# SHI-Labs/Prompt-Free-Diffusion

Hardware: NVIDIA H100
Metric: 512x512 images/sec @ 50 DDIM steps (higher is better)
Workload: dtype fp16

## Files before the change

### pfd_b200/autokl.py

```python
from __future__ import annotations

from typing import Optional

import torch
import torch.nn as nn

from . import native as nv
from .modules import Container, Conv2d, GroupNorm, pk_conv3, pk_conv3_small, pk_lin, pk_mat, pk_norm


def Normalize(c):
    return GroupNorm(32, c, eps=1e-6, affine=True)


class ResnetBlock(nn.Module):

    def __init__(self, in_channels, out_channels=None):
        super().__init__()
        out_channels = out_channels or in_channels
        self.in_channels, self.out_channels = in_channels, out_channels
        self.norm1 = Normalize(in_channels)
        self.conv1 = Conv2d(in_channels, out_channels, 3, padding=1)
        self.norm2 = Normalize(out_channels)
        self.dropout = nn.Dropout(0.0)
        self.conv2 = Conv2d(out_channels, out_channels, 3, padding=1)
        if in_channels != out_channels:
            self.nin_shortcut = Conv2d(in_channels, out_channels, 1)


class AttnBlock(nn.Module):

    def __init__(self, c):
        super().__init__()
        self.in_channels = c
        self.norm = Normalize(c)
        self.q, self.k, self.v, self.proj_out = Conv2d(c, c, 1), Conv2d(c, c, 1), Conv2d(c, c, 1), Conv2d(c, c, 1)


class _Resample(nn.Module):
    def __init__(self, c, stride):
        super().__init__()
# ... 128 lines not shown
        h = run_vae_resnet(enc.mid.block_1, h)
        h = run_vae_attn(enc.mid.attn_1, h)
        h = run_vae_resnet(enc.mid.block_2, h)
        g, b = pk_norm(enc.norm_out)
        h = nv.groupnorm(h, g, b, enc.norm_out.eps, silu=True)
        w, b = pk_conv3(enc.conv_out)
        h = nv.conv3x3(h, w, b)
        wq, bq = pk_lin(self.quant_conv)
        mom = nv.conv1x1(h, wq, bq)
        zc = self.quant_conv.weight.shape[0] // 2
        if out_posterior:
            return DiagonalGaussianDistribution(mom, zc)
        noise = torch.randn((B, zc, mom.shape[1], mom.shape[2])).to(mom.device)
        return nv.vae_posterior(mom, zc, noise=noise, scale=post_scale, want=("sample",))["sample"]

    @torch.no_grad()
    def decode(self, z: torch.Tensor, pre_scale: float = 1.0) -> torch.Tensor:
        dec = self.decoder
        B, Cz, H, W = z.shape
        nv.gn_reset()
        zc = nv.nchw_to_nhwc(z if z.dtype == torch.float32 else z.to(torch.float16), cpad=8)
        wq, bq = pk_lin(self.post_quant_conv)
        h = nv.linear(zc.reshape(B * H * W, 8), wq, bq, alpha=pre_scale).reshape(B, H, W, 8)
        w, b = cached_conv_in(dec.conv_in, Cz)
        h = nv.conv3x3_im2col(h, w, b)
        h = run_vae_resnet(dec.mid.block_1, h)
        h = run_vae_attn(dec.mid.attn_1, h)
        h = run_vae_resnet(dec.mid.block_2, h)
        for lvl in reversed(range(dec.num_resolutions)):
            up = dec.up[lvl]
            for rb in up.block:
                h = run_vae_resnet(rb, h)
            if lvl != 0:
                w, b = pk_conv3(up.upsample.conv)
                h = nv.conv3x3(nv.upsample2x(h), w, b)
        g, b = pk_norm(dec.norm_out)
        h = nv.groupnorm(h, g, b, dec.norm_out.eps, silu=True)
        w, b = pk_conv3(dec.conv_out)
        h = nv.conv3x3(h, w, b)
        return nv.nhwc_to_nchw(h, dec.out_ch, mul=0.5, add=0.5, lo=0.0, hi=1.0)

    def forward(self, z):
        return self.decode(z)


class DiagonalGaussianDistribution(object):

    def __init__(self, moments: torch.Tensor, zc: int):
        self._mom, self._zc = moments, zc
        o = nv.vae_posterior(moments, zc, want=("mean", "logvar", "std"))
        self.mean, self.logvar, self.std = o["mean"], o["logvar"], o["std"]
        self.deterministic = False

    def sample(self):
        noise = torch.randn(self.mean.shape).to(self.mean.device)
        return nv.vae_posterior(self._mom, self._zc, noise=noise, want=("sample",))["sample"]

    def mode(self):
        return self.mean


def cached_conv_in(conv: Conv2d, cz: int):
    from .modules import cached, fp16

    def build():
        o = conv.weight.shape[0]
        w = torch.zeros((o, 3, 3, 8), device=conv.weight.device, dtype=torch.float16)
        w[..., :cz] = fp16(conv.weight).permute(0, 2, 3, 1)
# ... 3 lines not shown
```

### pfd_b200/csrc/gemm_tc.cu

```cuda
#include <cuda.h>
#include <cuda_fp16.h>
#include <cuda_runtime.h>
#include <math.h>
#include <string.h>

#include "../../include/pfd_b200.h"
#include "common.h"
#include "ptx.cuh"
#include "wgmma.cuh"

namespace pfd {

constexpr int BM = 128;
constexpr int BK = 64;
constexpr int WG_K = 16;
constexpr int GEMM_THREADS = 384;
constexpr int STAGE_A_BYTES = BM * BK * 2;
constexpr int SMEM_BUDGET = 232448;
constexpr int SMEM_FIXED = 1024 + 256;

struct alignas(64) GemmParams {
  CUtensorMap tmA[PFD_MAX_SEG];
  CUtensorMap tmB;
  int nseg;
  int taps[PFD_MAX_SEG];
  int chunks[PFD_MAX_SEG];
  int a_c[PFD_MAX_SEG];
  int stride;
  int tap_off;
  int bw, bh, bn;
  int tiles_w, tiles_h, tiles_nb, n_tiles;
  int W, H, NB, N;
  int b_batched;
  int num_kb;
  int splits;
  int kb_per_split;
  float* ws;
  float alpha;
  int act;
  const __half* bias;
  const __half* rowadd;
  const __half* residual;
  __half* out;
  long long so_n1, so_n0, so_y, so_x, so_c1, so_c0;
  long long rowadd_ld;
  int ndiv, cdiv;
  int vec_ok;
};

constexpr int STORE_THREADS = 96;

template <int BN>
struct GemmCfg {
  static constexpr int STAGE_B_BYTES = BN * BK * 2;
  static constexpr int STAGE_BYTES = STAGE_A_BYTES + STAGE_B_BYTES;
  static constexpr int C_PITCH = BN * 2 + 16;
  static constexpr int C_BYTES = BM * C_PITCH + 2 * BM * 8;
  static constexpr int RAW_STAGES = (SMEM_BUDGET - SMEM_FIXED - C_BYTES) / STAGE_BYTES;
  static constexpr int STAGES = RAW_STAGES > 8 ? 8 : RAW_STAGES;
  static constexpr int SMEM_BYTES = STAGES * STAGE_BYTES + C_BYTES + SMEM_FIXED;
  static constexpr int CONSUMER_REGS = BN >= 256 ? 224 : 208;
  static constexpr int PRODUCER_REGS = BN >= 256 ? 56 : 88;
  static constexpr int STORE_BATCH = BN >= 256 ? 4 : 8;
  static constexpr bool BIAS_EARLY = BN < 256;
// ... 40 lines not shown
  lo = fmaf(lo, alpha, h2lo(bias));
  hi = fmaf(hi, alpha, h2hi(bias));
  if (rowadd) {
    lo += h2lo(ra);
    hi += h2hi(ra);
  }
  if (act != PFD_ACT_NONE) {
    lo = act_apply(lo, act);
    hi = act_apply(hi, act);
  }
}

__device__ __forceinline__ __half2 geglu_pair(const float* v, const float* g, float alpha, uint32_t bv, uint32_t bg) {
  const __half2 a = __floats2half2_rn(fmaf(v[0], alpha, h2lo(bv)), fmaf(v[1], alpha, h2hi(bv)));
  const float2 gf = __half22float2(__floats2half2_rn(fmaf(g[0], alpha, h2lo(bg)), fmaf(g[1], alpha, h2hi(bg))));
  return __hmul2(a, __floats2half2_rn(gelu_sig(gf.x), gelu_sig(gf.y)));
}

struct WorkItem {
  int tile, kb0, kb1, slot;
};
__device__ __forceinline__ bool gemm_work(const GemmParams& p, int wi, int total_tiles, WorkItem& w) {
  const int G = gridDim.x, c = blockIdx.x;
  const int work = c + wi * G;
  if (work >= total_tiles * p.splits) return false;
  w.tile = work % total_tiles;
  w.slot = work / total_tiles;
  w.kb0 = w.slot * p.kb_per_split;
  w.kb1 = min(p.num_kb, w.kb0 + p.kb_per_split);
  return true;
}

struct TileOrigin {
  int x0, y0, n0, lbw, lbh;
};
__device__ __forceinline__ TileOrigin tile_origin(const GemmParams& p, int m_tile) {
  TileOrigin o;
  o.x0 = (m_tile % p.tiles_w) * p.bw;
  o.y0 = ((m_tile / p.tiles_w) % p.tiles_h) * p.bh;
  o.n0 = (m_tile / (p.tiles_w * p.tiles_h)) * p.bn;
  o.lbw = __ffs(p.bw) - 1;
  o.lbh = __ffs(p.bh) - 1;
  return o;
}
struct TileRow {
  int x, y, n;
  bool valid;
};
__device__ __forceinline__ TileRow tile_row(const GemmParams& p, const TileOrigin& o, int row) {
  TileRow r;
  r.x = o.x0 + (row & (p.bw - 1));
  r.y = o.y0 + ((row >> o.lbw) & (p.bh - 1));
  r.n = o.n0 + (row >> (o.lbw + o.lbh));
  r.valid = (r.x < p.W) && (r.y < p.H) && (r.n < p.NB);
  return r;
}
__device__ __forceinline__ long long out_row_off(const GemmParams& p, const TileRow& r) {
  return (long long)(r.n / p.ndiv) * p.so_n1 + (long long)(r.n % p.ndiv) * p.so_n0 + (long long)r.y * p.so_y +
         (long long)r.x * p.so_x;
}
__device__ __forceinline__ long long out_col_off(const GemmParams& p, int c) {
  return p.cdiv >= p.N ? (long long)c * p.so_c0 : (long long)(c / p.cdiv) * p.so_c1 + (long long)(c % p.cdiv) * p.so_c0;
}

template <int BN>
__device__ __forceinline__ void gemm_load_bias(const GemmParams& p, int tile, uint32_t (&bias)[BN / 8]) {
  const int col0 = (tile % p.n_tiles) * BN + 2 * (threadIdx.x & 3);
#pragma unroll
  for (int j = 0; j < BN / 8; ++j) bias[j] = (p.bias && col0 + 8 * j < p.N) ? ldg_h2(p.bias + col0 + 8 * j) : 0u;
}

template <int BN, bool GEGLU>
__device__ __forceinline__ void gemm_stage_tile(const GemmParams& p, const float (&acc)[BN / 2],
                                                const uint32_t (&bias)[BN / 8], int cw, int tile, uint8_t* cbuf) {
  constexpr int C_PITCH = GemmCfg<BN>::C_PITCH;
  const int wl = (threadIdx.x >> 5) & 3, lane = threadIdx.x & 31;
  const int n_tile = tile % p.n_tiles;
  const TileOrigin org = tile_origin(p, tile / p.n_tiles);
  const int n_out = GEGLU ? p.N / 2 : p.N;
  const int col_base = n_tile * (GEGLU ? BN / 2 : BN);
  const int cq = 2 * (lane & 3);
  int rows[2];
  bool valid[2];
  const __half* rowadd_row[2];
#pragma unroll
  for (int i = 0; i < 2; ++i) {
    rows[i] = cw * 64 + wl * 16 + (lane >> 2) + 8 * i;
    const TileRow r = tile_row(p, org, rows[i]);
    valid[i] = r.valid;
    rowadd_row[i] = (p.rowadd && r.valid) ? p.rowadd + (long long)r.n * p.rowadd_ld : nullptr;
  }
  auto put = [&](int i, int c, __half2 h) {
// ... 21 lines not shown
    uint32_t ra[2][JB];
#pragma unroll
    for (int jj = 0; jj < JB; ++jj) {
      const int col = col_base + 8 * (j0 + jj) + cq;
#pragma unroll
      for (int i = 0; i < 2; ++i) ra[i][jj] = (rowadd_row[i] && col < n_out) ? ldg_h2(rowadd_row[i] + col) : 0u;
    }
#pragma unroll
    for (int jj = 0; jj < JB; ++jj) {
      const int j = j0 + jj;
      if (col_base + 8 * j + cq >= n_out) continue;
#pragma unroll
      for (int i = 0; i < 2; ++i) {
        if (!valid[i]) continue;
        float v0 = acc[4 * j + 2 * i], v1 = acc[4 * j + 2 * i + 1];
        epi_pair(v0, v1, alpha, bias[j], rowadd_row[i] != nullptr, ra[i][jj], act);
        put(i, 8 * j + cq, __floats2half2_rn(v0, v1));
      }
    }
  }
}

template <int BN, bool GEGLU>
__device__ __forceinline__ void gemm_store_tile(const GemmParams& p, int tile, const uint8_t* cbuf, long long* rowoff,
                                                uint32_t c_full, uint32_t parity) {
  constexpr int C_PITCH = GemmCfg<BN>::C_PITCH;
  constexpr int STORE_BATCH = GemmCfg<BN>::STORE_BATCH;
  constexpr int CPR = (GEGLU ? BN / 2 : BN) / 8;
  constexpr int RPP = STORE_THREADS / CPR;
  constexpr int NPASS = (BM + RPP - 1) / RPP;
  const int t = threadIdx.x - 32;
  const int n_tile = tile % p.n_tiles;
  const TileOrigin org = tile_origin(p, tile / p.n_tiles);
  const bool line_tile = p.bw == BM;
  if (!line_tile) {
#pragma unroll 1
    for (int row = t; row < BM; row += STORE_THREADS) {
      const TileRow r = tile_row(p, org, row);
      rowoff[row] = r.valid ? out_row_off(p, r) : -1;
    }
    asm volatile("bar.sync 2, %0;" ::"n"(STORE_THREADS) : "memory");
  }
  const int ch = t % CPR, r0 = t / CPR;
  const int col = n_tile * CPR * 8 + 8 * ch;
  const bool col_ok = r0 < RPP && col < (GEGLU ? p.N / 2 : p.N);
  const long long col_off = out_col_off(p, col);
  const bool add_res = p.residual && !GEGLU;
  const uint8_t* const src = cbuf + r0 * C_PITCH + ch * 16;

  auto store_rows = [&](auto row_off) {
    uint4 res[STORE_BATCH];
    auto load_batch = [&](int pass0) {
#pragma unroll
      for (int b = 0; b < STORE_BATCH; ++b) {
        const int row = r0 + (pass0 + b) * RPP;
        const long long off = (col_ok && row < BM) ? row_off(row) : -1;
        if (off >= 0) res[b] = __ldg(reinterpret_cast<const uint4*>(p.residual + off));
      }
    };
    if (add_res) load_batch(0);
    mbar_wait(c_full, parity);
#pragma unroll 1
    for (int pass0 = 0; pass0 < NPASS; pass0 += STORE_BATCH) {
#pragma unroll
      for (int b = 0; b < STORE_BATCH; ++b) {
        const int row = r0 + (pass0 + b) * RPP;
        const long long off = (col_ok && row < BM) ? row_off(row) : -1;
        if (off < 0) continue;
        uint4 v = *reinterpret_cast<const uint4*>(src + (pass0 + b) * (RPP * C_PITCH));
        if (add_res) {
          __half2* h = reinterpret_cast<__half2*>(&v);
          const __half2* r = reinterpret_cast<const __half2*>(&res[b]);
#pragma unroll
          for (int k = 0; k < 4; ++k) h[k] = __hadd2(h[k], r[k]);
        }
        *reinterpret_cast<uint4*>(p.out + off) = v;
      }
      if (add_res && pass0 + STORE_BATCH < NPASS) load_batch(pass0 + STORE_BATCH);
    }
  };

  if (line_tile) {
    const int rows_in = p.W - org.x0;
    TileRow first;
    first.x = org.x0; first.y = org.y0; first.n = org.n0;
    const long long base = out_row_off(p, first) + col_off;
    const long long so_x = p.so_x;
    store_rows([&](int row) { return row < rows_in ? base + row * so_x : -1ll; });
  } else {
    store_rows([&](int row) {
      const long long ro = rowoff[row];
      return ro >= 0 ? ro + col_off : -1ll;
    });
  }
}

template <int BN>
__device__ __forceinline__ void gemm_epilogue(const GemmParams& p, const float (&acc)[BN / 2], int cw, int tile,
                                              int split, int m_tiles) {
  const int wl = (threadIdx.x >> 5) & 3, lane = threadIdx.x & 31;
  const int n_tile = tile % p.n_tiles;
  const int m_tile = tile / p.n_tiles;
  const TileOrigin org = tile_origin(p, m_tile);
  const bool geglu = (p.act == PFD_ACT_GEGLU);
  const int n_out = geglu ? p.N / 2 : p.N;
  const int col_base = n_tile * (geglu ? BN / 2 : BN);
  const int cq = 2 * (lane & 3);
  int rows[2];
  bool valid[2];
  long long row_off[2];
  const __half* rowadd_row[2];
#pragma unroll
  for (int i = 0; i < 2; ++i) {
    const int row = cw * 64 + wl * 16 + (lane >> 2) + 8 * i;
    rows[i] = row;
    const TileRow r = tile_row(p, org, row);
    valid[i] = r.valid;
    row_off[i] = out_row_off(p, r);
    rowadd_row[i] = (p.rowadd && valid[i]) ? p.rowadd + (long long)r.n * p.rowadd_ld : nullptr;
// ... 68 lines not shown
  constexpr int STAGES = Cfg::STAGES;
  extern __shared__ uint8_t smem_raw[];

  const uint32_t raw_addr = smem_u32(smem_raw);
  const uint32_t base = (raw_addr + 1023u) & ~1023u;
  const uint32_t smemA = base;
  const uint32_t smemB = base + STAGES * STAGE_A_BYTES;
  const uint32_t cbuf_off = base - raw_addr + STAGES * Cfg::STAGE_BYTES;
  uint8_t* const cbuf = smem_raw + cbuf_off;
  long long* const rowoff = reinterpret_cast<long long*>(cbuf + BM * Cfg::C_PITCH);
  const uint32_t bars = base + STAGES * Cfg::STAGE_BYTES + Cfg::C_BYTES;
  auto full_bar = [&](int s) { return bars + 8u * s; };
  auto empty_bar = [&](int s) { return bars + 8u * (STAGES + s); };
  const uint32_t c_full = bars + 16u * STAGES, c_empty = c_full + 8u;

  const int wg = threadIdx.x >> 7;
  const bool staged = p.vec_ok && p.splits == 1;

  if (threadIdx.x == 0) {
    for (int s = 0; s < p.nseg; ++s) tma_prefetch_desc(&p.tmA[s]);
    tma_prefetch_desc(&p.tmB);
    for (int s = 0; s < STAGES; ++s) {
      mbar_init(full_bar(s), 1);
      mbar_init(empty_bar(s), 8);
    }
    mbar_init(c_full, 8);
    mbar_init(c_empty, STORE_THREADS / 32);
    mbar_fence_init();
  }
  __syncthreads();
  pdl_wait();
  pdl_launch_dependents();

  const int m_tiles = p.tiles_w * p.tiles_h * p.tiles_nb;
  const int total_tiles = m_tiles * p.n_tiles;

  if (wg == 0) {
    setmaxnreg_dec<Cfg::PRODUCER_REGS>();
    if (threadIdx.x >= 32 && staged) {
      uint32_t c_phase = 0;
      WorkItem w;
      for (int wi = 0; gemm_work(p, wi, total_tiles, w); ++wi) {
        if (p.act == PFD_ACT_GEGLU) gemm_store_tile<BN, true>(p, w.tile, cbuf, rowoff + (c_phase ? BM : 0), c_full, c_phase);
        else gemm_store_tile<BN, false>(p, w.tile, cbuf, rowoff + (c_phase ? BM : 0), c_full, c_phase);
        __syncwarp();
        if ((threadIdx.x & 31) == 0) mbar_arrive(c_empty);
        c_phase ^= 1u;
      }
    } else if (threadIdx.x == 0) {
      int stage = 0;
      uint32_t phase = 0;
      WorkItem w;
      for (int wi = 0; gemm_work(p, wi, total_tiles, w); ++wi) {
        const int tile = w.tile, kb_begin = w.kb0, kb_end = w.kb1;
        const int n_tile = tile % p.n_tiles;
        const int m_tile = tile / p.n_tiles;
        const int tx = m_tile % p.tiles_w;
        const int ty = (m_tile / p.tiles_w) % p.tiles_h;
        const int tn = m_tile / (p.tiles_w * p.tiles_h);
        const int x0 = tx * p.bw * p.stride;
        const int y0 = ty * p.bh * p.stride;
        const int n0 = tn * p.bn;
        const int bcoord = p.b_batched ? n0 : 0;
        int kofs = 0;
        int kbi = 0;
        for (int s = 0; s < p.nseg; ++s) {
          const int ntap = p.taps[s];
          for (int t = 0; t < ntap; ++t) {
            const int dy = (ntap == 9) ? (t / 3 - 1 + p.tap_off) : 0;
            const int dx = (ntap == 9) ? (t % 3 - 1 + p.tap_off) : 0;
            for (int j = 0; j < p.chunks[s]; ++j, ++kbi) {
              if (kbi < kb_begin || kbi >= kb_end) continue;
              mbar_wait(empty_bar(stage), phase ^ 1u);
              mbar_expect_tx(full_bar(stage), Cfg::STAGE_BYTES);
              tma_load_4d(smemA + stage * STAGE_A_BYTES, &p.tmA[s], full_bar(stage), j * BK, x0 + dx, y0 + dy, n0);
              tma_load_3d(smemB + stage * Cfg::STAGE_B_BYTES, &p.tmB, full_bar(stage), kofs + j * BK, n_tile * BN,
                          bcoord);
              if (++stage == STAGES) {
                stage = 0;
                phase ^= 1u;
              }
            }
            kofs += p.a_c[s];
          }
        }
      }
    }
  } else {
    setmaxnreg_inc<Cfg::CONSUMER_REGS>();
    const int cw = wg - 1;
    const bool arrive_lane = (threadIdx.x & 31) == 0;
    int stage = 0;
    uint32_t phase = 0, c_phase = 0;
    float acc[BN / 2];
    WorkItem w;
    for (int wi = 0; gemm_work(p, wi, total_tiles, w); ++wi) {
      const int nkb = w.kb1 - w.kb0;
      uint32_t bias[BN / 8];
      if (Cfg::BIAS_EARLY && staged) gemm_load_bias<BN>(p, w.tile, bias);
      int prev = -1;
      for (int kb = 0; kb < nkb; ++kb) {
        mbar_wait(full_bar(stage), phase);
        const uint64_t adesc = make_sw128_kmajor_desc(smemA + stage * STAGE_A_BYTES + cw * 64 * 128);
// ... 2 lines not shown
#pragma unroll
        for (int k = 0; k < BK / WG_K; ++k)
          Wgmma<BN>::ss(acc, adesc + 2u * k, bdesc + 2u * k, (kb | k) != 0 ? 1u : 0u);
        wgmma_commit();
        wgmma_wait<1>();
        if (prev >= 0 && arrive_lane) mbar_arrive(empty_bar(prev));
        prev = stage;
        if (++stage == STAGES) {
          stage = 0;
          phase ^= 1u;
        }
      }
      wgmma_wait<0>();
      if (prev >= 0 && arrive_lane) mbar_arrive(empty_bar(prev));
      if (staged) {
        if (!Cfg::BIAS_EARLY) gemm_load_bias<BN>(p, w.tile, bias);
        mbar_wait(c_empty, c_phase ^ 1u);
        if (p.act == PFD_ACT_GEGLU) gemm_stage_tile<BN, true>(p, acc, bias, cw, w.tile, cbuf);
        else gemm_stage_tile<BN, false>(p, acc, bias, cw, w.tile, cbuf);
        __syncwarp();
        if (arrive_lane) mbar_arrive(c_full);
        c_phase ^= 1u;
      } else {
        gemm_epilogue<BN>(p, acc, cw, w.tile, w.slot, m_tiles);
      }
    }
  }
}

__global__ void __launch_bounds__(256)
splitk_finish_kernel(const __grid_constant__ GemmParams p) {
  pdl_wait();
  pdl_launch_dependents();
  const int m_tiles = p.tiles_w * p.tiles_h * p.tiles_nb;
  const long long rows_pad = (long long)m_tiles * BM;
  const int vecs = p.N / 8;
  const long long total = rows_pad * vecs;
  for (long long i = (long long)blockIdx.x * blockDim.x + threadIdx.x; i < total; i += (long long)gridDim.x * blockDim.x) {
    const int v = (int)(i % vecs);
    const long long prow = i / vecs;
    const TileRow r = tile_row(p, tile_origin(p, (int)(prow / BM)), (int)(prow % BM));
    if (!r.valid) continue;
    const int col = v * 8;
    float acc[8];
#pragma unroll
    for (int k = 0; k < 8; ++k) acc[k] = 0.f;
    for (int s = 0; s < p.splits; ++s) {
      const float4* src = reinterpret_cast<const float4*>(p.ws + ((long long)s * rows_pad + prow) * p.N + col);
      const float4 a = __ldg(src), b = __ldg(src + 1);
      acc[0] += a.x; acc[1] += a.y; acc[2] += a.z; acc[3] += a.w;
      acc[4] += b.x; acc[5] += b.y; acc[6] += b.z; acc[7] += b.w;
    }
    uint4 bv = make_uint4(0, 0, 0, 0), rv = bv;
    if (p.bias) bv = __ldg(reinterpret_cast<const uint4*>(p.bias + col));
    if (p.rowadd) rv = __ldg(reinterpret_cast<const uint4*>(p.rowadd + (long long)r.n * p.rowadd_ld + col));
    const uint32_t* b2 = &bv.x;
    const uint32_t* r2 = &rv.x;
#pragma unroll
    for (int k = 0; k < 4; ++k)
      epi_pair(acc[2 * k], acc[2 * k + 1], p.alpha, b2[k], p.rowadd != nullptr, r2[k], p.act);
    const long long row_off = out_row_off(p, r);
    if (p.vec_ok) {
      const long long off = row_off + out_col_off(p, col);
      uint4 o;
      __half2* oh = reinterpret_cast<__half2*>(&o);
#pragma unroll
      for (int k = 0; k < 4; ++k) oh[k] = __floats2half2_rn(acc[2 * k], acc[2 * k + 1]);
// ... 19 lines not shown
constexpr size_t SPLITK_WS_BYTES = (64ull << 20) - 4096;

static inline long long cdivll(long long a, long long b) { return (a + b - 1) / b; }

template <int BN>
static int launch_gemm(const GemmParams& p, int grid, cudaStream_t stream) {
  using Cfg = GemmCfg<BN>;
  static int trace = -1;
  if (trace < 0) {
    const char* e = getenv("PFD_GEMM_TRACE");
    trace = (e && e[0] == '1') ? 1 : 0;
  }
  if (trace)
    fprintf(stderr, "GEMMTRACE M=%lld N=%d K=%d nseg=%d taps=%d stride=%d act=%d bias=%d res=%d rowadd=%d BN=%d "
            "splits=%d grid=%d batched=%d vec=%d plain=%d\n", (long long)p.W * p.H * p.NB, p.N, p.num_kb * BK,
            p.nseg, p.taps[0], p.stride, p.act, p.bias != nullptr, p.residual != nullptr, p.rowadd != nullptr, BN,
            p.splits, grid, p.b_batched, p.vec_ok, (int)(p.cdiv >= p.N));
  if (int rc = smem_opt_in<gemm_wgmma_kernel<BN>>(Cfg::SMEM_BYTES, "gemm_wgmma_kernel")) return rc;
  launch_k(gemm_wgmma_kernel<BN>, dim3(grid), dim3(GEMM_THREADS), Cfg::SMEM_BYTES, stream, p);
  return check_launch("pfd_gemm_f16");
}

}

using namespace pfd;

extern "C" PFD_API int pfd_gemm_f16(const pfd_gemm_desc* d) {
  if (!d) return set_error("pfd_gemm_f16: null descriptor");
  if (d->nseg < 1 || d->nseg > PFD_MAX_SEG) return set_error("pfd_gemm_f16: nseg %d out of range", d->nseg);
  if (d->N <= 0 || d->N % 8) return set_error("pfd_gemm_f16: N=%d must be a positive multiple of 8", d->N);
  if (d->K % 8) return set_error("pfd_gemm_f16: K pitch %lld must be a multiple of 8", (long long)d->K);
  if (d->W <= 0 || d->H <= 0 || d->NB <= 0) return set_error("pfd_gemm_f16: empty output raster");
  if (d->stride != 1 && d->stride != 2) return set_error("pfd_gemm_f16: stride %d unsupported", d->stride);
  if (d->tap_off != 0 && d->tap_off != 1) return set_error("pfd_gemm_f16: tap_off %d unsupported", d->tap_off);
  if (!d->out || !d->b_ptr) return set_error("pfd_gemm_f16: null out/b pointer");
  long long ktot = 0;
  for (int s = 0; s < d->nseg; ++s) {
    if (d->taps[s] != 1 && d->taps[s] != 9) return set_error("pfd_gemm_f16: taps[%d]=%d", s, d->taps[s]);
    if (d->a_c[s] <= 0 || d->a_c[s] % 8) return set_error("pfd_gemm_f16: a_c[%d]=%d must be a multiple of 8", s, d->a_c[s]);
    if (!d->a_ptr[s]) return set_error("pfd_gemm_f16: a_ptr[%d] is null", s);
    if ((reinterpret_cast<uintptr_t>(d->a_ptr[s]) & 15) || (d->a_sx[s] % 8) || (d->a_sy[s] % 8) || (d->a_sn[s] % 8))
      return set_error("pfd_gemm_f16: A segment %d not 16-byte aligned/strided", s);
    ktot += (long long)d->taps[s] * d->a_c[s];
  }
  if (ktot > d->K) return set_error("pfd_gemm_f16: segments cover K=%lld > pitch %lld", ktot, (long long)d->K);
  if (reinterpret_cast<uintptr_t>(d->b_ptr) & 15) return set_error("pfd_gemm_f16: B not 16-byte aligned");
  const bool geglu = d->act == PFD_ACT_GEGLU;

  GemmParams p;
  memset(&p, 0, sizeof(p));
  p.nseg = d->nseg;
  p.stride = d->stride;
  p.tap_off = d->tap_off;
  p.W = d->W; p.H = d->H; p.NB = d->NB; p.N = d->N;
  p.b_batched = d->b_batch_stride != 0;
  p.alpha = d->alpha;
  p.act = d->act;
  p.bias = static_cast<const __half*>(d->bias);
  p.rowadd = static_cast<const __half*>(d->rowadd);
  p.residual = static_cast<const __half*>(d->residual);
  p.rowadd_ld = d->rowadd_ld > 0 ? d->rowadd_ld : d->N;
  p.out = static_cast<__half*>(d->out);
  p.so_n1 = d->so_n1; p.so_n0 = d->so_n0; p.so_y = d->so_y; p.so_x = d->so_x;
  p.so_c1 = d->so_c1; p.so_c0 = d->so_c0;
  p.ndiv = d->ndiv > 0 ? d->ndiv : 1;
  p.cdiv = d->cdiv > 0 ? d->cdiv : (1 << 30);
  p.vec_ok = (d->so_c0 == 1) && (p.cdiv % 8 == 0) && (d->so_n1 % 8 == 0) && (d->so_n0 % 8 == 0) &&
             (d->so_y % 8 == 0) && (d->so_x % 8 == 0) && (d->so_c1 % 8 == 0) &&
             ((reinterpret_cast<uintptr_t>(d->out) & 15) == 0) &&
             ((reinterpret_cast<uintptr_t>(d->residual) & 15) == 0);
  if ((reinterpret_cast<uintptr_t>(d->bias) & 15) || (reinterpret_cast<uintptr_t>(d->rowadd) & 15) || (d->rowadd_ld % 8))
    return set_error("pfd_gemm_f16: bias/rowadd must be 16-byte aligned");

  int bw = 128, bh = 1, bn = 1;
  if (!p.b_batched) {
    long long best = -1;
    for (int cw = 128; cw >= 1; cw >>= 1) {
      if (cw * d->stride > 256) continue;
      for (int ch = 128 / cw; ch >= 1; ch >>= 1) {
        if (ch * d->stride > 256) continue;
        int cn = 128 / (cw * ch);
        long long cost = cdivll(d->W, cw) * cdivll(d->H, ch) * cdivll(d->NB, cn);
        if (best < 0 || cost < best) {
          best = cost; bw = cw; bh = ch; bn = cn;
        }
      }
    }
  }
  p.bw = bw; p.bh = bh; p.bn = bn;
  p.tiles_w = (int)cdivll(d->W, bw);
  p.tiles_h = (int)cdivll(d->H, bh);
  p.tiles_nb = (int)cdivll(d->NB, bn);
  const long long m_tiles = (long long)p.tiles_w * p.tiles_h * p.tiles_nb;

  bool short_k_plain = !p.b_batched && !geglu;
  int kb_count = 0;
  for (int s = 0; s < d->nseg; ++s) {
    if (d->taps[s] != 1) short_k_plain = false;
    kb_count += d->taps[s] * ((d->a_c[s] + BK - 1) / BK);
  }
  short_k_plain = short_k_plain && kb_count <= 40;
  const int cands[5] = {256, 192, 160, 128, 64};
  int BNsel = 128;
  double best_cost = -1;
  const int sms = plan_sms();
  for (int i = 0; i < 5; ++i) {
    const int bn_c = cands[i];
    if (geglu && (d->N % bn_c)) continue;
    if (d->bn_force && d->bn_force != bn_c) continue;
    if (short_k_plain && !d->bn_force && bn_c != 64) continue;
    const long long nt = cdivll(d->N, bn_c);
    const long long tiles = m_tiles * nt;
    const double waves = (double)cdivll(tiles, sms);
    const double cost = waves * (bn_c + 24);
    if (best_cost < 0 || cost < best_cost - 1e-9) {
      best_cost = cost; BNsel = bn_c;
    }
  }
  if (best_cost < 0) return set_error("pfd_gemm_f16: no valid N tile (bn_force=%d, N=%d, geglu=%d)", d->bn_force, d->N, (int)geglu);
  p.n_tiles = (int)cdivll(d->N, BNsel);
  p.splits = 1;

  int num_kb = 0;
  for (int s = 0; s < d->nseg; ++s) {
    p.taps[s] = d->taps[s];
    p.a_c[s] = d->a_c[s];
// ... 8 lines not shown
  p.num_kb = num_kb;
  p.kb_per_split = num_kb;
  cudaStream_t st = static_cast<cudaStream_t>(d->stream);
  float* const skws = static_cast<float*>(device_scratch(SCRATCH_SPLITK, SPLITK_WS_BYTES, 0, st));
  if (!geglu && !d->bn_force && num_kb >= 32 && !deterministic()) {
    int bn_sk = 128;
    const int sk_cands[4] = {256, 192, 160, 128};
    for (int i = 0; i < 4; ++i)
      if (d->N % sk_cands[i] == 0) {
        bn_sk = sk_cands[i];
        break;
      }
    const long long nt_sk = cdivll(d->N, bn_sk);
    const long long tiles_sk = m_tiles * nt_sk;
    if (tiles_sk * 2 <= sms) {
      int splits = (int)(sms / tiles_sk);
      if (splits > 8) splits = 8;
      if (splits > num_kb / 8) splits = num_kb / 8;
      const size_t need = (size_t)splits * (size_t)m_tiles * BM * (size_t)d->N * sizeof(float);
      if (splits >= 2 && need <= SPLITK_WS_BYTES) {
        float* ws = skws;
        if (ws) {
          BNsel = bn_sk;
          p.n_tiles = (int)nt_sk;
          p.splits = splits;
          p.kb_per_split = (num_kb + splits - 1) / splits;
          p.splits = (num_kb + p.kb_per_split - 1) / p.kb_per_split;
          p.ws = ws;
        }
      }
    }
  }
  {
    const long long nbatch = p.b_batched ? d->NB : 1;
    cuuint64_t dims[3] = {(cuuint64_t)d->K, (cuuint64_t)d->N, (cuuint64_t)nbatch};
    const long long bs = p.b_batched ? d->b_batch_stride : (long long)d->K * d->N;
    cuuint64_t strides[2] = {(cuuint64_t)d->K * 2, (cuuint64_t)bs * 2};
    cuuint32_t box[3] = {(cuuint32_t)BK, (cuuint32_t)BNsel, 1};
    cuuint32_t estr[3] = {1, 1, 1};
    if (int rc = encode_tensor_map_f16(&p.tmB, d->b_ptr, 3, dims, strides, box, estr, "B")) return rc;
  }
  const long long total = m_tiles * p.n_tiles * p.splits;
  int grid = (int)(total < sms ? total : sms);
  int rc;
  switch (BNsel) {
    case 64: rc = launch_gemm<64>(p, grid, st); break;
    case 128: rc = launch_gemm<128>(p, grid, st); break;
    case 160: rc = launch_gemm<160>(p, grid, st); break;
    case 192: rc = launch_gemm<192>(p, grid, st); break;
    default: rc = launch_gemm<256>(p, grid, st); break;
  }
  if (rc || p.splits == 1) return rc;
  const long long vec_items = m_tiles * BM * (long long)(d->N / 8);
  long long fgrid = (vec_items + 255) / 256;
  if (fgrid > 8LL * sms) fgrid = 8LL * sms;
  launch_k(splitk_finish_kernel, dim3((unsigned)fgrid), dim3(256), 0, st, p);
  return check_launch("pfd_gemm_f16(split-K finish)");
}
```

### pfd_b200/modules.py

```python
from __future__ import annotations

from typing import Callable, Optional, Sequence, Tuple

import torch
import torch.nn as nn

from .graphs import generation, watch


class _Holder:
    def forward(self, *a, **k):
        raise RuntimeError(f"{type(self).__name__} is a parameter holder: pfd_b200 computes through "
                           "the CUDA C-ABI kernels only (no torch fallback)")


class Conv2d(_Holder, nn.Conv2d):
    pass


class Linear(_Holder, nn.Linear):
    pass


class GroupNorm(_Holder, nn.GroupNorm):
# ... 58 lines not shown
def pad_cols(w: torch.Tensor, mult: int = 8) -> torch.Tensor:
    k = w.shape[1]
    if k % mult == 0:
        return w
    pad = torch.zeros((w.shape[0], mult - k % mult), device=w.device, dtype=w.dtype)
    return torch.cat([w, pad], 1).contiguous()


def pack_conv(weight: torch.Tensor, cin: Optional[int] = None) -> torch.Tensor:
    w = fp16(weight)
    o, i, kh, kw = w.shape
    if cin is not None and cin > i:
        w = torch.cat([w, w.new_zeros((o, cin - i, kh, kw))], 1)
    return w.permute(0, 2, 3, 1).reshape(o, -1).contiguous()


def pk_conv3(conv: nn.Conv2d, skip: Optional[nn.Conv2d] = None) -> Tuple[torch.Tensor, Optional[torch.Tensor]]:
    def build():
        w = pack_conv(conv.weight)
        b = fp16(conv.bias)
        if skip is not None:
            ws = fp16(skip.weight).reshape(skip.weight.shape[0], -1)
            w = torch.cat([w, ws], 1).contiguous()
            if skip.bias is not None:
                b = (conv.bias.detach().float() + skip.bias.detach().float()).to(torch.float16).contiguous()
        if w.shape[0] % 8:
            w = pad_rows(w)
            b = pad_rows(b) if b is not None else None
        return w, b
    params = [conv.weight, conv.bias] + ([skip.weight, skip.bias] if skip is not None else [])
    return cached(conv, "conv3" + ("+skip" if skip is not None else ""), params, build)


def pk_conv3_small(conv: nn.Conv2d) -> Tuple[torch.Tensor, Optional[torch.Tensor]]:
    def build():
        w = pad_cols(pack_conv(conv.weight))
        b = fp16(conv.bias)
        if w.shape[0] % 8:
            w, b = pad_rows(w), (pad_rows(b) if b is not None else None)
        return w, b
    return cached(conv, "conv3s", [conv.weight, conv.bias], build)


def pk_mat(mod: nn.Module, weight: torch.Tensor, bias: Optional[torch.Tensor], key: str = "mat",
           rows: Optional[slice] = None) -> Tuple[torch.Tensor, Optional[torch.Tensor]]:
    def build():
        w = fp16(weight).reshape(weight.shape[0], -1)
        b = fp16(bias)
        if rows is not None:
            w = w[rows].contiguous()
            b = b[rows].contiguous() if b is not None else None
        if w.shape[1] % 8:
            w = pad_cols(w)
        if w.shape[0] % 8:
            w, b = pad_rows(w), (pad_rows(b) if b is not None else None)
        return w, b
    return cached(mod, key, [weight, bias], build)


def pk_lin(lin: nn.Module, key: str = "mat"):
    return pk_mat(lin, lin.weight, lin.bias, key)


def pk_norm(norm: nn.Module) -> Tuple[torch.Tensor, torch.Tensor]:
    return cached(norm, "norm", [norm.weight, norm.bias], lambda: (fp16(norm.weight), fp16(norm.bias)))

# ... 4 lines not shown
```

### pfd_b200/native.py

```python
from __future__ import annotations

import ctypes
import os
import re
from ctypes import POINTER, c_char_p, c_float, c_int32, c_int64, c_uint32, c_void_p
from typing import Dict, List, Optional, Sequence, Tuple

import torch

_HERE = os.path.dirname(os.path.abspath(__file__))
LIB_PATH = os.environ.get("PFD_B200_LIB") or os.path.join(_HERE, "libpfd_b200.so")
HEADER = os.path.join(_HERE, os.pardir, "include", "pfd_b200.h")

PFD_MAX_SEG = 3
ACT_NONE, ACT_SILU, ACT_GELU, ACT_RELU, ACT_GEGLU = 0, 1, 2, 3, 4
PFD_KSAMPLER_NCOEF = 6
PFD_HED_MAX_SIDES = 5
PFD_PIDINET_SIDE_PARAMS = 161
PFD_MLSD_TOPK = 200
PFD_OPENPOSE_MAX_PEAKS = 128
PFD_OPENPOSE_MAX_PERSONS = 17 * PFD_OPENPOSE_MAX_PEAKS


class GemmDesc(ctypes.Structure):
# ... 220 lines not shown

def pack_geglu(w: torch.Tensor, b: Optional[torch.Tensor]):
    n2 = w.shape[0]
    inner = n2 // 2
    bn = geglu_tile(n2)
    h = bn // 2
    idx = torch.arange(n2, device=w.device).reshape(n2 // bn, 2, h)
    tile = torch.arange(n2 // bn, device=w.device).reshape(-1, 1)
    j = torch.arange(h, device=w.device).reshape(1, -1)
    src = torch.stack([tile * h + j, inner + tile * h + j], dim=1).reshape(-1)
    wp = w.index_select(0, src).contiguous()
    bp = b.index_select(0, src).contiguous() if b is not None else None
    return wp, bp, bn


def conv3x3(x: torch.Tensor, w: torch.Tensor, bias: Optional[torch.Tensor] = None, *, stride: int = 1,
            rowadd: Optional[torch.Tensor] = None, act: int = ACT_NONE,
            residual: Optional[torch.Tensor] = None, out: Optional[torch.Tensor] = None,
            skip: Sequence[torch.Tensor] = (), tap_off: int = 0) -> torch.Tensor:
    NB, H, W, C = x.shape
    Ho, Wo = (H - 1 - tap_off) // stride + 1, (W - 1 - tap_off) // stride + 1
    N = w.shape[0]
    if out is None:
        out = torch.empty((NB, Ho, Wo, N), device=x.device, dtype=torch.float16)
    segs = [(x, 9, C, (x.stride(2), x.stride(1), x.stride(0)))]
    for s in skip:
        segs.append((s, 1, s.shape[3], (s.stride(2), s.stride(1), s.stride(0))))
    gemm_raw(segs, in_w=W, in_h=H, stride=stride, W=Wo, H=Ho, NB=NB, w=w, N=N, K=w.stride(0), act=act,
             bias=bias, rowadd=rowadd, residual=residual, out=out,
             so=(out.stride(0), 0, out.stride(1), out.stride(2), 0, 1), tap_off=tap_off)
    return out


def conv1x1(x: torch.Tensor, w: torch.Tensor, bias: Optional[torch.Tensor] = None, *, act: int = ACT_NONE,
            residual: Optional[torch.Tensor] = None, out: Optional[torch.Tensor] = None,
            x2: Optional[torch.Tensor] = None) -> torch.Tensor:
    NB, H, W, C = x.shape
    N = w.shape[0]
    if out is None:
        out = torch.empty((NB, H, W, N), device=x.device, dtype=torch.float16)
    r = residual.reshape(NB * H * W, -1) if residual is not None else None
    linear(x.reshape(NB * H * W, C), w, bias, act=act, residual=r, out=out.reshape(NB * H * W, N),
           x2=None if x2 is None else x2.reshape(NB * H * W, -1))
    return out


def conv1x1_into(x: torch.Tensor, w: torch.Tensor, bias: Optional[torch.Tensor], out: torch.Tensor, *,
                 act: int = ACT_NONE) -> torch.Tensor:
    NB, H, W, C = x.shape
    gemm_raw([(x, 1, C, (x.stride(2), x.stride(1), x.stride(0)))], in_w=W, in_h=H, stride=1, W=W, H=H, NB=NB, w=w,
             N=w.shape[0], K=w.stride(0), act=act, bias=bias, out=out,
             so=(out.stride(0), 0, out.stride(1), out.stride(2), 0, 1))
    return out


def bmm_nt(a: torch.Tensor, b: torch.Tensor, *, out: torch.Tensor, so, ndiv: int = 1, cdiv: int = 0,
           alpha: float = 1.0) -> None:
    B, M, K = a.shape
    N = b.shape[1]
    gemm_raw([(a, 1, K, (a.stride(1), a.stride(1) * M, a.stride(0)))], in_w=M, in_h=1, stride=1, W=M,
             H=1, NB=B, w=b, N=N, K=b.stride(1), b_batch_stride=b.stride(0), alpha=alpha, out=out,
             so=so, ndiv=ndiv, cdiv=cdiv)


_GN_SLOT_BYTES = 64 * 32 * 16 + 256
_GN_SLOTS = 256
# ... 664 lines not shown
```

### pfd_b200/unet.py

```python
from __future__ import annotations

from typing import Dict, List, Optional, Sequence, Tuple

import torch
import torch.nn as nn

from . import native as nv
from . import attention as att
from .attention import attend, ceil8, project_heads, project_heads_fused, project_vt_swapped
from .modules import (Conv2d, GroupNorm, IndexedSequential, LayerNorm, Linear, cached, pk_conv3,
                      pk_conv3_small, pk_lin, pk_mat, pk_norm)


class ResBlock(nn.Module):

    def __init__(self, channels, emb_channels, dropout=0.0, out_channels=None, **_):
        super().__init__()
        self.channels = channels
        self.out_channels = out_channels or channels
        self.in_layers = IndexedSequential(GroupNorm(32, channels), nn.SiLU(),
                                           Conv2d(channels, self.out_channels, 3, padding=1))
        self.emb_layers = IndexedSequential(nn.SiLU(), Linear(emb_channels, self.out_channels))
        self.out_layers = IndexedSequential(GroupNorm(32, self.out_channels), nn.SiLU(), nn.Dropout(p=dropout),
                                            Conv2d(self.out_channels, self.out_channels, 3, padding=1))
        if self.out_channels == channels:
            self.skip_connection = nn.Identity()
        else:
            self.skip_connection = Conv2d(channels, self.out_channels, 1)


class Downsample(nn.Module):

    def __init__(self, channels, out_channels=None):
        super().__init__()
        self.channels = channels
        self.out_channels = out_channels or channels
        self.op = Conv2d(channels, self.out_channels, 3, stride=2, padding=1)


class Upsample(nn.Module):

    def __init__(self, channels, out_channels=None):
        super().__init__()
        self.channels = channels
# ... 229 lines not shown
                add_d(ResBlock(ch + ich, ted, dropout, out_channels=model_channels * mult))
                ch = model_channels * mult
                if ds in attention_resolutions:
                    add_c(ch)
            if level != 0:
                add_d(Upsample(ch, out_channels=ch))
                ds //= 2
        add_d(IndexedSequential(GroupNorm(32, ch), nn.SiLU(), Conv2d(model_channels, out_channels, 3, padding=1)))
        self.o_order = list(order)
        self.layer_order = self.i_order + self.m_order + self.o_order
        self.parameter_group = {'global': self.time_embed, 'data': self.data_blocks,
                                'context': self.context_blocks}

    def get_d_head_n_heads(self, ch):
        if self.num_head_channels is None:
            return ch // self.num_heads, self.num_heads
        return self.num_head_channels, ch // self.num_head_channels

    def resblocks(self) -> List[ResBlock]:
        return [blk[0] for blk in self.data_blocks if isinstance(blk[0], ResBlock)]

    def prepare_context(self, context: torch.Tensor) -> List[Tuple[torch.Tensor, torch.Tensor]]:
        return [context_kv(cb[0], context) for cb in self.context_blocks]

    def run_data_block(self, idx: int, h, h2, embs: Dict[int, torch.Tensor]):
        layer = self.data_blocks[idx][0]
        if isinstance(layer, ResBlock):
            return run_resblock(layer, h, h2, embs[idx])
        assert h2 is None
        if isinstance(layer, Downsample):
            w, b = pk_conv3(layer.op)
            return nv.conv3x3(h, w, b, stride=2)
        if isinstance(layer, Upsample):
            w, b = pk_conv3(layer.conv)
            return nv.conv3x3(nv.upsample2x(h), w, b)
        if isinstance(layer, IndexedSequential):
            g, b = pk_norm(layer[0])
            hn = nv.groupnorm(h, g, b, layer[0].eps, silu=True)
            w, bb = pk_conv3(layer[2])
            return nv.conv3x3(hn, w, bb)
        if isinstance(layer, Conv2d):
            w, b = pk_conv3_small(layer)
            return nv.conv3x3_im2col(h, w, b)
        raise RuntimeError(f"unknown data block {type(layer)}")

    def apply(self, x: torch.Tensor, timesteps: torch.Tensor, context: torch.Tensor,
              control: Optional[List[torch.Tensor]] = None,
              kv: Optional[List[Tuple[torch.Tensor, torch.Tensor]]] = None,
              mixed_contexts: Optional[List[Tuple[torch.Tensor, float]]] = None) -> torch.Tensor:
        x = x.to(torch.float16)
        context = context.to(torch.float16).contiguous()
        B = x.shape[0]
        nv.gn_reset()
        silu_emb = time_embed_silu(self.time_embed, timesteps, self.model_channels)
        rbs = [i for i, blk in enumerate(self.data_blocks) if isinstance(blk[0], ResBlock)]
        emb_list = batched_emb_layers(self, [self.data_blocks[i][0] for i in rbs], silu_emb)
        embs = dict(zip(rbs, emb_list))
        if kv is None and mixed_contexts is None:
            kv = self.prepare_context(context)
        ccs = list(control) if control is not None else None
        h = nv.nchw_to_nhwc(x)
        h2 = None
        hs: List[torch.Tensor] = []
        di = ci = 0
        for lt in self.i_order + self.m_order + ['__mid__'] + self.o_order:
            if lt == 'd':
                h = self.run_data_block(di, h, h2, embs)
                h2 = None
# ... 26 lines not shown
```

Baseline: 3.826.

## Fuse nearest upsample into 3x3 conv via four-phase 2x2 sub-pixel weights

Replaces nearest-2x upsample followed by a 3x3 conv with a single GEMM that treats each of the four output phases as a 2x2 conv over the low-resolution input, using precombined per-phase weights. This avoids materializing the upsampled tensor and cuts conv MACs from 9 to 4 taps per output. The GEMM kernel gains an 'up' mode that selects the phase-specific weight batch, offsets the taps and scatters rows to interleaved output positions. The combined weights are rounded to fp16 after summing in double, so results may differ slightly from the original path, and the scattered stores lose the contiguous line-tile path.

```diff
diff --git a/pfd_b200/autokl.py b/pfd_b200/autokl.py
--- a/pfd_b200/autokl.py
+++ b/pfd_b200/autokl.py
@@ -6,7 +6,8 @@
 import torch.nn as nn
 
 from . import native as nv
-from .modules import Container, Conv2d, GroupNorm, pk_conv3, pk_conv3_small, pk_lin, pk_mat, pk_norm
+from .modules import (Container, Conv2d, GroupNorm, pk_conv3, pk_conv3_small, pk_conv3_up, pk_lin, pk_mat,
+                      pk_norm)
 
 
 def Normalize(c):
@@ -201,8 +202,8 @@
             for rb in up.block:
                 h = run_vae_resnet(rb, h)
             if lvl != 0:
-                w, b = pk_conv3(up.upsample.conv)
-                h = nv.conv3x3(nv.upsample2x(h), w, b)
+                w, b = pk_conv3_up(up.upsample.conv)
+                h = nv.upsample_conv3x3(h, w, b)
         g, b = pk_norm(dec.norm_out)
         h = nv.groupnorm(h, g, b, dec.norm_out.eps, silu=True)
         w, b = pk_conv3(dec.conv_out)
diff --git a/pfd_b200/csrc/gemm_tc.cu b/pfd_b200/csrc/gemm_tc.cu
--- a/pfd_b200/csrc/gemm_tc.cu
+++ b/pfd_b200/csrc/gemm_tc.cu
@@ -30,6 +30,7 @@
   int tap_off;
   int bw, bh, bn;
   int tiles_w, tiles_h, tiles_nb, n_tiles;
+  int up;
   int W, H, NB, N;
   int b_batched;
   int num_kb;
@@ -136,19 +137,21 @@
 }
 
 struct TileOrigin {
-  int x0, y0, n0, lbw, lbh;
+  int x0, y0, n0, ph, lbw, lbh;
 };
 __device__ __forceinline__ TileOrigin tile_origin(const GemmParams& p, int m_tile) {
   TileOrigin o;
   o.x0 = (m_tile % p.tiles_w) * p.bw;
   o.y0 = ((m_tile / p.tiles_w) % p.tiles_h) * p.bh;
-  o.n0 = (m_tile / (p.tiles_w * p.tiles_h)) * p.bn;
+  const int tn = m_tile / (p.tiles_w * p.tiles_h);
+  o.ph = p.up ? tn / p.tiles_nb : 0;
+  o.n0 = (tn - o.ph * p.tiles_nb) * p.bn;
   o.lbw = __ffs(p.bw) - 1;
   o.lbh = __ffs(p.bh) - 1;
   return o;
 }
 struct TileRow {
-  int x, y, n;
+  int x, y, n, ph;
   bool valid;
 };
 __device__ __forceinline__ TileRow tile_row(const GemmParams& p, const TileOrigin& o, int row) {
@@ -156,12 +159,16 @@
   r.x = o.x0 + (row & (p.bw - 1));
   r.y = o.y0 + ((row >> o.lbw) & (p.bh - 1));
   r.n = o.n0 + (row >> (o.lbw + o.lbh));
+  r.ph = o.ph;
   r.valid = (r.x < p.W) && (r.y < p.H) && (r.n < p.NB);
   return r;
 }
+__device__ __forceinline__ long long out_row_off(const GemmParams& p, int n, int y, int x) {
+  return (long long)(n / p.ndiv) * p.so_n1 + (long long)(n % p.ndiv) * p.so_n0 + (long long)y * p.so_y +
+         (long long)x * p.so_x;
+}
 __device__ __forceinline__ long long out_row_off(const GemmParams& p, const TileRow& r) {
-  return (long long)(r.n / p.ndiv) * p.so_n1 + (long long)(r.n % p.ndiv) * p.so_n0 + (long long)r.y * p.so_y +
-         (long long)r.x * p.so_x;
+  return out_row_off(p, r.n, (r.y << p.up) + (r.ph >> 1), (r.x << p.up) + (r.ph & 1));
 }
 __device__ __forceinline__ long long out_col_off(const GemmParams& p, int c) {
   return p.cdiv >= p.N ? (long long)c * p.so_c0 : (long long)(c / p.cdiv) * p.so_c1 + (long long)(c % p.cdiv) * p.so_c0;
@@ -249,7 +256,7 @@
   const int t = threadIdx.x - 32;
   const int n_tile = tile % p.n_tiles;
   const TileOrigin org = tile_origin(p, tile / p.n_tiles);
-  const bool line_tile = p.bw == BM;
+  const bool line_tile = p.bw == BM && !p.up;
   if (!line_tile) {
 #pragma unroll 1
     for (int row = t; row < BM; row += STORE_THREADS) {
@@ -299,9 +306,7 @@
 
   if (line_tile) {
     const int rows_in = p.W - org.x0;
-    TileRow first;
-    first.x = org.x0; first.y = org.y0; first.n = org.n0;
-    const long long base = out_row_off(p, first) + col_off;
+    const long long base = out_row_off(p, org.n0, org.y0, org.x0) + col_off;
     const long long so_x = p.so_x;
     store_rows([&](int row) { return row < rows_in ? base + row * so_x : -1ll; });
   } else {
@@ -436,7 +441,7 @@
   pdl_wait();
   pdl_launch_dependents();
 
-  const int m_tiles = p.tiles_w * p.tiles_h * p.tiles_nb;
+  const int m_tiles = p.tiles_w * p.tiles_h * p.tiles_nb << (2 * p.up);
   const int total_tiles = m_tiles * p.n_tiles;
 
   if (wg == 0) {
@@ -462,17 +467,24 @@
         const int tx = m_tile % p.tiles_w;
         const int ty = (m_tile / p.tiles_w) % p.tiles_h;
         const int tn = m_tile / (p.tiles_w * p.tiles_h);
+        const int ph = tn / p.tiles_nb;
         const int x0 = tx * p.bw * p.stride;
         const int y0 = ty * p.bh * p.stride;
-        const int n0 = tn * p.bn;
-        const int bcoord = p.b_batched ? n0 : 0;
+        const int n0 = (tn % p.tiles_nb) * p.bn;
+        const int bcoord = p.b_batched ? n0 : ph;
         int kofs = 0;
         int kbi = 0;
         for (int s = 0; s < p.nseg; ++s) {
           const int ntap = p.taps[s];
           for (int t = 0; t < ntap; ++t) {
-            const int dy = (ntap == 9) ? (t / 3 - 1 + p.tap_off) : 0;
-            const int dx = (ntap == 9) ? (t % 3 - 1 + p.tap_off) : 0;
+            int dy = 0, dx = 0;
+            if (ntap == 9) {
+              dy = t / 3 - 1 + p.tap_off;
+              dx = t % 3 - 1 + p.tap_off;
+            } else if (ntap == 4) {
+              dy = (t >> 1) + (ph >> 1) - 1;
+              dx = (t & 1) + (ph & 1) - 1;
+            }
             for (int j = 0; j < p.chunks[s]; ++j, ++kbi) {
               if (kbi < kb_begin || kbi >= kb_end) continue;
               mbar_wait(empty_bar(stage), phase ^ 1u);
@@ -541,7 +553,7 @@
 splitk_finish_kernel(const __grid_constant__ GemmParams p) {
   pdl_wait();
   pdl_launch_dependents();
-  const int m_tiles = p.tiles_w * p.tiles_h * p.tiles_nb;
+  const int m_tiles = p.tiles_w * p.tiles_h * p.tiles_nb << (2 * p.up);
   const long long rows_pad = (long long)m_tiles * BM;
   const int vecs = p.N / 8;
   const long long total = rows_pad * vecs;
@@ -627,11 +639,18 @@
   if (d->K % 8) return set_error("pfd_gemm_f16: K pitch %lld must be a multiple of 8", (long long)d->K);
   if (d->W <= 0 || d->H <= 0 || d->NB <= 0) return set_error("pfd_gemm_f16: empty output raster");
   if (d->stride != 1 && d->stride != 2) return set_error("pfd_gemm_f16: stride %d unsupported", d->stride);
+  if (!d->out || !d->b_ptr) return set_error("pfd_gemm_f16: null out/b pointer");
+  bool taps4 = false;
+  for (int s = 0; s < d->nseg; ++s) taps4 = taps4 || d->taps[s] == 4;
+  if (taps4 && (d->stride != 1 || d->tap_off != 0 || d->b_batch_stride != 0))
+    return set_error("pfd_gemm_f16: 2x2 taps need stride 1, tap_off 0 and shared weights (got %d, %d, %lld)",
+                     d->stride, d->tap_off, (long long)d->b_batch_stride);
   if (d->tap_off != 0 && d->tap_off != 1) return set_error("pfd_gemm_f16: tap_off %d unsupported", d->tap_off);
-  if (!d->out || !d->b_ptr) return set_error("pfd_gemm_f16: null out/b pointer");
   long long ktot = 0;
   for (int s = 0; s < d->nseg; ++s) {
-    if (d->taps[s] != 1 && d->taps[s] != 9) return set_error("pfd_gemm_f16: taps[%d]=%d", s, d->taps[s]);
+    if (d->taps[s] != 1 && d->taps[s] != 4 && d->taps[s] != 9)
+      return set_error("pfd_gemm_f16: taps[%d]=%d", s, d->taps[s]);
+    if (taps4 && d->taps[s] == 9) return set_error("pfd_gemm_f16: 2x2 and 3x3 tap segments in one call");
     if (d->a_c[s] <= 0 || d->a_c[s] % 8) return set_error("pfd_gemm_f16: a_c[%d]=%d must be a multiple of 8", s, d->a_c[s]);
     if (!d->a_ptr[s]) return set_error("pfd_gemm_f16: a_ptr[%d] is null", s);
     if ((reinterpret_cast<uintptr_t>(d->a_ptr[s]) & 15) || (d->a_sx[s] % 8) || (d->a_sy[s] % 8) || (d->a_sn[s] % 8))
@@ -686,7 +705,8 @@
   p.tiles_w = (int)cdivll(d->W, bw);
   p.tiles_h = (int)cdivll(d->H, bh);
   p.tiles_nb = (int)cdivll(d->NB, bn);
-  const long long m_tiles = (long long)p.tiles_w * p.tiles_h * p.tiles_nb;
+  p.up = taps4 ? 1 : 0;
+  const long long m_tiles = (long long)p.tiles_w * p.tiles_h * p.tiles_nb << (2 * p.up);
 
   bool short_k_plain = !p.b_batched && !geglu;
   int kb_count = 0;
@@ -761,7 +781,7 @@
     }
   }
   {
-    const long long nbatch = p.b_batched ? d->NB : 1;
+    const long long nbatch = p.b_batched ? d->NB : p.up ? 4 : 1;
     cuuint64_t dims[3] = {(cuuint64_t)d->K, (cuuint64_t)d->N, (cuuint64_t)nbatch};
     const long long bs = p.b_batched ? d->b_batch_stride : (long long)d->K * d->N;
     cuuint64_t strides[2] = {(cuuint64_t)d->K * 2, (cuuint64_t)bs * 2};
diff --git a/pfd_b200/modules.py b/pfd_b200/modules.py
--- a/pfd_b200/modules.py
+++ b/pfd_b200/modules.py
@@ -114,6 +114,29 @@
     return cached(conv, "conv3" + ("+skip" if skip is not None else ""), params, build)
 
 
+_UP_TAPS = ((((1, 0, 0), (0, 1, 1))), (((1, 1, 0), (0, 0, 1))))
+
+
+def up_phase_weights(weight: torch.Tensor) -> torch.Tensor:
+    w = weight.detach().double()
+    r = torch.tensor(_UP_TAPS, dtype=torch.float64, device=w.device)
+    return torch.einsum("pak,qbl,oikl->pqoiab", r, r, w).reshape(4, *w.shape[:2], 2, 2)
+
+
+def pk_conv3_up(conv: nn.Conv2d) -> Tuple[torch.Tensor, Optional[torch.Tensor]]:
+    def build():
+        w = up_phase_weights(fp16(conv.weight))
+        o, i = w.shape[1:3]
+        return half_rn(w.permute(0, 1, 3, 4, 2).reshape(4, o, 4 * i)).contiguous(), fp16(conv.bias)
+    return cached(conv, "conv3up", [conv.weight, conv.bias], build)
+
+
+def half_rn(x: torch.Tensor) -> torch.Tensor:
+    _, e = torch.frexp(x)
+    q = torch.pow(2.0, (torch.clamp(e - 1, min=-14) - 10).double())
+    return (torch.round(x / q) * q).to(torch.float16)
+
+
 def pk_conv3_small(conv: nn.Conv2d) -> Tuple[torch.Tensor, Optional[torch.Tensor]]:
     def build():
         w = pad_cols(pack_conv(conv.weight))
diff --git a/pfd_b200/native.py b/pfd_b200/native.py
--- a/pfd_b200/native.py
+++ b/pfd_b200/native.py
@@ -276,6 +276,15 @@
     return out
 
 
+def upsample_conv3x3(x: torch.Tensor, w4: torch.Tensor, bias: Optional[torch.Tensor] = None) -> torch.Tensor:
+    NB, H, W, C = x.shape
+    N = w4.shape[1]
+    out = torch.empty((NB, 2 * H, 2 * W, N), device=x.device, dtype=torch.float16)
+    gemm_raw([(x, 4, C, (x.stride(2), x.stride(1), x.stride(0)))], in_w=W, in_h=H, stride=1, W=W, H=H, NB=NB, w=w4,
+             N=N, K=w4.stride(1), bias=bias, out=out, so=(out.stride(0), 0, out.stride(1), out.stride(2), 0, 1))
+    return out
+
+
 def conv1x1(x: torch.Tensor, w: torch.Tensor, bias: Optional[torch.Tensor] = None, *, act: int = ACT_NONE,
             residual: Optional[torch.Tensor] = None, out: Optional[torch.Tensor] = None,
             x2: Optional[torch.Tensor] = None) -> torch.Tensor:
diff --git a/pfd_b200/unet.py b/pfd_b200/unet.py
--- a/pfd_b200/unet.py
+++ b/pfd_b200/unet.py
@@ -9,7 +9,7 @@
 from . import attention as att
 from .attention import attend, ceil8, project_heads, project_heads_fused, project_vt_swapped
 from .modules import (Conv2d, GroupNorm, IndexedSequential, LayerNorm, Linear, cached, pk_conv3,
-                      pk_conv3_small, pk_lin, pk_mat, pk_norm)
+                      pk_conv3_small, pk_conv3_up, pk_lin, pk_mat, pk_norm)
 
 
 class ResBlock(nn.Module):
@@ -305,8 +305,8 @@
             w, b = pk_conv3(layer.op)
             return nv.conv3x3(h, w, b, stride=2)
         if isinstance(layer, Upsample):
-            w, b = pk_conv3(layer.conv)
-            return nv.conv3x3(nv.upsample2x(h), w, b)
+            w, b = pk_conv3_up(layer.conv)
+            return nv.upsample_conv3x3(h, w, b)
         if isinstance(layer, IndexedSequential):
             g, b = pk_norm(layer[0])
             hn = nv.groupnorm(h, g, b, layer[0].eps, silu=True)
```

Measured after the change: 3.915 (median of 6 runs). +2.3%, better.
